# andompesta/nodeembedding-to-communityembedding

Measured on AMD Instinct MI355X. Metric: SGNS pair-updates/sec at d=128, 1M-node graph, higher is better.
Workload: dtype f32

## Files before the change

### nodeembedding-to-communityembedding_amd/csrc/come_sgns_impl.h

```cpp
#pragma once
#include <hip/hip_runtime.h>
#include <stdint.h>

#include "come_internal.h"
#include "come_wave.h"

namespace come {

static __constant__ float c_exp_table[kExpTableSize];

struct LcgLane {
    uint64_t a, c;
};

__device__ inline LcgLane lcg_lane_constants(int k) {
    uint64_t a = 1, c = 0;
    for (int i = 0; i < k; ++i) {
        a = (a * kLcgMul) & kLcgMask;
        c = (c * kLcgMul + kLcgAdd) & kLcgMask;
    }
    return {a, c};
}

__device__ inline uint64_t lcg_next(uint64_t s) { return (s * kLcgMul + kLcgAdd) & kLcgMask; }

struct LcgTable {
    uint64_t a[64], c[64];
};
constexpr LcgTable make_lcg_table() {
    LcgTable t{};
    uint64_t a = 1, c = 0;
    for (int k = 0; k < 64; ++k) {
        t.a[k] = a;
        t.c[k] = c;
        a = (a * kLcgMul) & kLcgMask;
        c = (c * kLcgMul + kLcgAdd) & kLcgMask;
    }
    return t;
}
static __constant__ LcgTable c_lcg = make_lcg_table();
constexpr LcgTable kLcgHost = make_lcg_table();
constexpr uint64_t kLcgA64 = (kLcgHost.a[63] * kLcgMul) & kLcgMask;
constexpr uint64_t kLcgC64 = (kLcgHost.c[63] * kLcgMul + kLcgAdd) & kLcgMask;

struct LcgFromTable {
    int lane;
};
__device__ inline uint64_t lcg_state_of(uint64_t base, const LcgLane &lc) {
    return (lc.a * base + lc.c) & kLcgMask;
}
__device__ inline uint64_t lcg_state_of(uint64_t base, const LcgFromTable &lt) {
    return (c_lcg.a[lt.lane] * base + c_lcg.c[lt.lane]) & kLcgMask;
}

__device__ inline uint32_t table_slot(uint64_t s, uint64_t m, uint32_t d) {
    const uint32_t x = (uint32_t)(s >> 16);
    if (d == 0) return x;
    return (uint32_t)__umul64hi(m * (uint64_t)x, (uint64_t)d);
}

struct PackedWord {
    uint32_t base;
    uint32_t unused;
    uint64_t bits;
};

template <class Args>
__device__ inline uint32_t table_value(const Args &a, uint32_t slot) {
    if (a.packed) {
        const uint4 w = reinterpret_cast<const uint4 *>(a.table)[slot >> 6];
        const uint64_t bits = ((uint64_t)w.w << 32) | w.z;
        const uint64_t mask = (2ull << (slot & 63)) - 1ull;
        return w.x + (uint32_t)__popcll(bits & mask);
    }
    return a.table[slot];
}

__device__ inline int uniform(int v) { return __builtin_amdgcn_readfirstlane(v); }
__device__ inline float uniformf(float v) {
    return __int_as_float(__builtin_amdgcn_readfirstlane(__float_as_int(v)));
}
__device__ inline uint64_t uniform64(uint64_t v) {
    const uint32_t lo = __builtin_amdgcn_readfirstlane((uint32_t)v);
    const uint32_t hi = __builtin_amdgcn_readfirstlane((uint32_t)(v >> 32));
    return ((uint64_t)hi << 32) | lo;
}
__device__ inline uint32_t readlane_u32(uint32_t v, int lane) {
    return (uint32_t)__builtin_amdgcn_readlane((int)v, lane);
}
__device__ inline uint64_t readlane_u64(uint64_t v, int lane) {
    const uint32_t lo = readlane_u32((uint32_t)v, lane);
    const uint32_t hi = readlane_u32((uint32_t)(v >> 32), lane);
    return ((uint64_t)hi << 32) | lo;
}

template <int VEC, bool FULL>
struct Row {
    float v[VEC];

    __device__ inline void load(const float *__restrict__ row, int lane, int d) {
#pragma unroll
        for (int i = 0; i < VEC; ++i) {
            const int e = lane + 64 * i;
            v[i] = (FULL || e < d) ? row[e] : 0.0f;
        }
    }

    __device__ inline void load_nt(const float *__restrict__ row, int lane, int d) {
#pragma unroll
        for (int i = 0; i < VEC; ++i) {
            const int e = lane + 64 * i;
            v[i] = (FULL || e < d) ? __builtin_nontemporal_load(row + e) : 0.0f;
        }
    }

    __device__ inline void load_fresh(const float *__restrict__ row, int lane, int d) {
#pragma unroll
        for (int i = 0; i < VEC; ++i) {
            const int e = lane + 64 * i;
            v[i] = (FULL || e < d) ? __hip_atomic_load(row + e, __ATOMIC_RELAXED,
                                                       __HIP_MEMORY_SCOPE_AGENT)
                                   : 0.0f;
        }
    }

    __device__ inline void load_as(const float *__restrict__ row, int lane, int d, bool fresh) {
        if (fresh) load_fresh(row, lane, d);
        else load(row, lane, d);
    }

    __device__ inline void store(float *__restrict__ row, int lane, int d) const {
#pragma unroll
        for (int i = 0; i < VEC; ++i) {
            const int e = lane + 64 * i;
            if (FULL || e < d) row[e] = v[i];
        }
    }

    __device__ inline void atomic_add(float *__restrict__ row, int lane, int d) const {
#pragma unroll
        for (int i = 0; i < VEC; ++i) {
            const int e = lane + 64 * i;
            if (FULL || e < d) atomicAdd(row + e, v[i]);
        }
    }
};

template <int VEC, bool FULL>
__device__ inline float lane_partial(const Row<VEC, FULL> &a, const Row<VEC, FULL> &b) {
    float p = 0.0f;
#pragma unroll
    for (int i = 0; i < VEC; ++i) p = __builtin_fmaf(a.v[i], b.v[i], p);
    return p;
}

__device__ inline float wave_sum(float p) {
    p = reduce_stage<0>(p);
    p = reduce_stage<1>(p);
    p = reduce_stage<2>(p);
    p = reduce_stage<3>(p);
    p = reduce_stage<4>(p);
    return reduce_stage<5>(p);
}

template <int N>
__device__ inline void wave_sum_n(float (&part)[N], int count) {
#define COME_STAGE(S)                                          \
    _Pragma("unroll") for (int k = 0; k < N; ++k) if (k < count) part[k] = reduce_stage<S>(part[k]);
    COME_STAGE(0) COME_STAGE(1) COME_STAGE(2) COME_STAGE(3) COME_STAGE(4) COME_STAGE(5)
#undef COME_STAGE
}

__device__ inline bool sigmoid_ref(float f, float *sig) {
    if (f <= -(float)kMaxExp || f >= (float)kMaxExp) return false;
    const int b = (int)(((double)f + 6.0) * 83.0);
    *sig = c_exp_table[b];
    return true;
}

__device__ inline bool sigmoid_tab(const float *tab, float f, float *sig) {
    if (f <= -(float)kMaxExp || f >= (float)kMaxExp) return false;
    const int b = (int)(((double)f + 6.0) * 83.0);
    *sig = tab[b];
    return true;
}

struct DrawBatch {
    uint32_t target;
    uint64_t base;
    int used;
};

template <class Args>
__device__ inline void draws_fill(DrawBatch &b, uint64_t state0, const LcgLane &lc,
                                  const Args &a, int count = 64) {
    b.base = state0;
    b.used = 0;
    b.target = 0;
    if ((int)(threadIdx.x & 63) < count) {
        const uint64_t s = (lc.a * state0 + lc.c) & kLcgMask;
        b.target = table_value(a, table_slot(s, a.fm.m, a.fm.d));
    }
}

__device__ inline uint64_t draws_state_at_used(const DrawBatch &b, const LcgLane &lc) {
    const uint64_t s = (lc.a * b.base + lc.c) & kLcgMask;
    if (b.used < 64) return uniform64(readlane_u64(s, b.used));
    return lcg_next(uniform64(readlane_u64(s, 63)));
}

struct DrawPipe {
    uint32_t t0, t1;
    uint64_t base0, base1;
    int used;

    template <class Args, class Lcg>
    __device__ inline uint32_t gather(uint64_t base, const Lcg &lc, const Args &a) {
        const uint64_t s = lcg_state_of(base, lc);
        return table_value(a, table_slot(s, a.fm.m, a.fm.d));
    }

    template <class Args, class Lcg>
    __device__ inline uint32_t gather_hot(uint64_t base, const Lcg &lc, const Args &a) {
        const uint32_t v = gather(base, lc, a);
        if (a.hot == nullptr || (int64_t)v >= a.V) return v;
        return v | (((a.hot[v >> 5] >> (v & 31)) & 1u) << 31);
    }
};


struct O2Args {
    float *node;
    float *ctx;
    const int32_t *walks;
    const uint64_t *seeds;
    const uint32_t *table;
    int64_t V;
    int64_t P;
    int L;
    int d;
    int window;
    int negative;
    float lr;
    float alpha;
    FastMod fm;
    int packed;
    int64_t *counter;
    unsigned long long *upd_count;
    int fresh;
    int wb_atomic;
    const uint32_t *hot;
};

template <class Args>
__device__ inline bool is_hot(const Args &a, int r) {
    return a.hot != nullptr && ((a.hot[(uint32_t)r >> 5] >> (r & 31)) & 1u);
}

__device__ inline int64_t next_unit(int64_t *counter, int64_t cur, int64_t stride, int lane) {
    if (!counter) return cur + stride;
    int64_t v = 0;
    if (lane == 0) v = (int64_t)atomicAdd((unsigned long long *)counter, 1ull);
    return (int64_t)uniform64((uint64_t)v);
}

__device__ inline uint64_t advance64_uniform(uint64_t base) {
    return (kLcgA64 * base + kLcgC64) & kLcgMask;
}
__device__ inline uint64_t advance64(uint64_t base, const LcgLane &lc) {
    const uint64_t s = (lc.a * base + lc.c) & kLcgMask;
    return lcg_next(uniform64(readlane_u64(s, 63)));
}

template <int VEC, bool FULL>
__device__ inline void atomic_add_delta(float *__restrict__ row, const Row<VEC, FULL> &cur,
                                        const Row<VEC, FULL> &orig, int lane, int d) {
    Row<VEC, FULL> delta;
#pragma unroll
    for (int e = 0; e < VEC; ++e) delta.v[e] = cur.v[e] - orig.v[e];
    delta.atomic_add(row, lane, d);
}

template <int VEC, bool FULL, int MAXN>
__device__ inline void o2_pair(const O2Args &a, DrawBatch &db, const LcgLane &lc, int lane, int ci,
                               Row<VEC, FULL> &pos, bool &pos_upd, Row<VEC, FULL> &in,
                               Row<VEC, FULL> &work, int &nupd) {
    using R = Row<VEC, FULL>;
    const int n = a.negative;
    const int d = a.d;
    if (n > 0 && db.used + n > 64) draws_fill(db, draws_state_at_used(db, lc), lc, a);
    int t[MAXN + 1];
    bool valid[MAXN + 1];
    t[0] = ci;
    valid[0] = true;
#pragma unroll
    for (int k = 1; k <= MAXN; ++k) {
        if (k <= n) {
            const int tk = (int)readlane_u32(db.target, db.used + k - 1);
            t[k] = tk;
            valid[k] = tk != ci && tk >= 0 && tk < a.V;
        } else {
            t[k] = -1;
            valid[k] = false;
        }
    }
    if (n > 0) db.used += n;

    R r[MAXN + 1], o[MAXN + 1];
#pragma unroll
    for (int k = 1; k <= MAXN; ++k)
        if (valid[k]) {
            r[k].load_as(a.ctx + (int64_t)t[k] * d, lane, d, a.fresh);
            o[k] = r[k];
        }

    float part[MAXN + 1];
    part[0] = lane_partial(in, pos);
#pragma unroll
    for (int k = 1; k <= MAXN; ++k) part[k] = valid[k] ? lane_partial(in, r[k]) : 0.0f;
    wave_sum_n(part, n + 1);

#pragma unroll
    for (int e = 0; e < VEC; ++e) work.v[e] = 0.0f;
    {
        float sig;
        if (sigmoid_ref(uniformf(part[0]), &sig)) {
            const float g = ((1.0f - sig) * a.lr) * a.alpha;
#pragma unroll
            for (int e = 0; e < VEC; ++e) {
                work.v[e] = __builtin_fmaf(g, pos.v[e], work.v[e]);
                pos.v[e] = __builtin_fmaf(g, in.v[e], pos.v[e]);
            }
            pos_upd = true;
            ++nupd;
        }
    }
    bool upd[MAXN + 1];
    upd[0] = false;
#pragma unroll
    for (int k = 1; k <= MAXN; ++k) {
        upd[k] = false;
        if (!valid[k]) continue;
        float f = part[k];
        int prev = -1;
#pragma unroll
        for (int q = 1; q < k; ++q)
            if (valid[q] && t[q] == t[k]) prev = q;
        if (prev >= 0) {
#pragma unroll
            for (int q = 1; q < k; ++q) {
                if (q == prev) {
                    r[k] = r[q];
                    f = upd[q] ? wave_sum(lane_partial(in, r[k])) : part[q];
                }
            }
        }
        f = uniformf(f);
        part[k] = f;
        float sig;
        if (!sigmoid_ref(f, &sig)) continue;
        const float g = ((0.0f - sig) * a.lr) * a.alpha;
#pragma unroll
        for (int e = 0; e < VEC; ++e) {
            work.v[e] = __builtin_fmaf(g, r[k].v[e], work.v[e]);
            r[k].v[e] = __builtin_fmaf(g, in.v[e], r[k].v[e]);
        }
        upd[k] = true;
        ++nupd;
    }
#pragma unroll
    for (int k = 1; k <= MAXN; ++k) {
        if (!upd[k]) continue;
        if (!a.wb_atomic && !is_hot(a, t[k])) {
            r[k].store(a.ctx + (int64_t)t[k] * d, lane, d);
            continue;
        }
        bool last = true;
#pragma unroll
        for (int q = k + 1; q <= MAXN; ++q)
            if (upd[q] && t[q] == t[k]) last = false;
        if (last) atomic_add_delta(a.ctx + (int64_t)t[k] * d, r[k], o[k], lane, d);
    }
#pragma unroll
    for (int e = 0; e < VEC; ++e) in.v[e] = in.v[e] + work.v[e];
}

template <int VEC, bool FULL, int MAXN>
__global__ void __launch_bounds__(256) k_sgns_o2(O2Args a) {
    using R = Row<VEC, FULL>;
    const int lane = threadIdx.x & 63;
    const int64_t waves_per_block = blockDim.x >> 6;
    const int64_t gw = (int64_t)blockIdx.x * waves_per_block + (threadIdx.x >> 6);
    const int64_t nwaves = (int64_t)gridDim.x * waves_per_block;
    const LcgLane lc = lcg_lane_constants(lane);
    const int d = a.d;
    const int path_len = a.L < kMaxSentenceLen ? a.L : kMaxSentenceLen;

    for (int64_t p = gw; p < a.P; p += nwaves) {
        const int32_t *__restrict__ idx = a.walks + p * (int64_t)a.L;
        DrawBatch db;
        db.used = 0;
        db.base = uniform64(a.seeds[p]);
        db.target = 0;
        if (a.negative > 0) draws_fill(db, db.base, lc, a);
        int nupd = 0;
        for (int i = 0; i < path_len; ++i) {
            const int ci = uniform(idx[i]);
            if (ci < 0 || ci >= a.V) continue;
            const int j0 = i - a.window < 0 ? 0 : i - a.window;
            const int j1 = i + a.window + 1 > path_len ? path_len : i + a.window + 1;
            for (int j = j0; j < j1; ++j) {
                if (j == i) continue;
                const int cj = uniform(idx[j]);
                if (cj < 0 || cj >= a.V) continue;
                R in, pos;
                in.load_as(a.node + (int64_t)cj * d, lane, d, a.fresh);
                pos.load_as(a.ctx + (int64_t)ci * d, lane, d, a.fresh);
                const R pos0 = pos;
                bool pos_upd = false;
                R work;
                o2_pair<VEC, FULL, MAXN>(a, db, lc, lane, ci, pos, pos_upd, in, work, nupd);
                if (pos_upd) {
                    if (a.wb_atomic || is_hot(a, ci))
                        atomic_add_delta(a.ctx + (int64_t)ci * d, pos, pos0, lane, d);
                    else
                        pos.store(a.ctx + (int64_t)ci * d, lane, d);
                }
                if (a.wb_atomic || is_hot(a, cj)) work.atomic_add(a.node + (int64_t)cj * d, lane, d);
                else in.store(a.node + (int64_t)cj * d, lane, d);
            }
        }
        if (a.upd_count && lane == 0 && nupd) atomicAdd(a.upd_count, (unsigned long long)nupd);
    }
}

template <int VEC, bool FULL, int MAXN>
__global__ void __launch_bounds__(128) k_sgns_o2_ring(O2Args a) {
    using R = Row<VEC, FULL>;
    extern __shared__ __attribute__((aligned(16))) float lds[];
    const int lane = threadIdx.x & 63;
    const int wib = threadIdx.x >> 6;
    const int64_t waves_per_block = blockDim.x >> 6;
    const int64_t gw = (int64_t)blockIdx.x * waves_per_block + wib;
    const int64_t nwaves = (int64_t)gridDim.x * waves_per_block;
    const LcgLane lc = lcg_lane_constants(lane);
    const int d = a.d;
    const int w = a.window;
    const int n = a.negative;
    const int RS = 2 * w + 1;
    const int path_len = a.L < kMaxSentenceLen ? a.L : kMaxSentenceLen;
    const int wave_floats = (RS * d + 3) & ~3;
    float *ring = lds + wib * wave_floats;
    auto valid_row = [&](int r) { return r >= 0 && r < a.V; };
    auto slot_add = [&](int s, int delta) {
        s += delta;
        if (s < 0) s += RS;
        if (s >= RS) s -= RS;
        return s;
    };

    for (int64_t p = a.counter ? next_unit(a.counter, 0, 0, lane) : gw; p < a.P;
         p = next_unit(a.counter, p, nwaves, lane)) {
        const int32_t *__restrict__ walk = a.walks + p * (int64_t)a.L;
        int wbase = 0;
        int c0 = lane < path_len ? walk[lane] : -1;
        int c1 = 64 + lane < path_len ? walk[64 + lane] : -1;
        auto idx_at = [&](int q) {
            if (q >= path_len) return -1;
            const int off = q - wbase;
            const int r = off < 64 ? __builtin_amdgcn_readlane(c0, off)
                                   : __builtin_amdgcn_readlane(c1, off - 64);
            return valid_row(r) ? r : -1;
        };
        DrawPipe dp;
        dp.used = 0;
        dp.base0 = uniform64(a.seeds[p]);
        dp.t0 = dp.t1 = 0;
        if (n > 0) {
            dp.t0 = dp.gather(dp.base0, lc, a);
            dp.base1 = advance64(dp.base0, lc);
            dp.t1 = dp.gather(dp.base1, lc, a);
        }
        auto take = [&](int k) -> int {
            const int q = dp.used + k;
            return (int)(q < 64 ? readlane_u32(dp.t0, q) : readlane_u32(dp.t1, q - 64));
        };
        auto advance = [&]() {
            if (n == 0) return;
            dp.used += n;
            if (dp.used >= 64) {
                dp.used -= 64;
                dp.t0 = dp.t1;
                dp.base0 = dp.base1;
                dp.base1 = advance64(dp.base1, lc);
                dp.t1 = dp.gather(dp.base1, lc, a);
            }
        };
        int tn[MAXN + 1];
        R rn[MAXN + 1];
        auto fetch_next = [&]() {
#pragma unroll
            for (int k = 1; k <= MAXN; ++k) {
                const int tk = k <= n ? take(k - 1) : -1;
                tn[k] = tk;
                rn[k].load(a.ctx + (int64_t)(valid_row(tk) ? tk : 0) * d, lane, d);
            }
        };
        fetch_next();

        int nupd = 0;
        int ids = -1;
        auto id_of = [&](int s) { return __builtin_amdgcn_readlane(ids, s); };
        auto alias_mask = [&](int id, int except) -> uint64_t {
            return __ballot(lane < RS && lane != except && ids == id);
        };
        auto set_id = [&](int s, int id) { ids = lane == s ? id : ids; };
        auto write_back = [&](int s, int id) {
            if (alias_mask(id, s) != 0) return;
            R row;
            row.load(ring + s * d, lane, d);
            row.store(a.node + (int64_t)id * d, lane, d);
        };
        auto enter_row = [&](int s, int id, const R &fetched) {
            const uint64_t m = alias_mask(id, s);
            if (m) {
                R row;
                row.load(ring + __builtin_ctzll(m) * d, lane, d);
                row.store(ring + s * d, lane, d);
            } else {
                fetched.store(ring + s * d, lane, d);
            }
            set_id(s, id);
        };
        for (int q = 0; q < w && q < path_len; ++q) {
            const int id = idx_at(q);
            if (id >= 0) {
                R row;
                row.load(a.node + (int64_t)id * d, lane, d);
                enter_row(q, id, row);
            }
        }
        R pos_n, ent_n;
        int pos_n_id = idx_at(0), ent_n_id = idx_at(w);
        pos_n.load(a.ctx + (int64_t)(pos_n_id >= 0 ? pos_n_id : 0) * d, lane, d);
        ent_n.load(a.node + (int64_t)(ent_n_id >= 0 ? ent_n_id : 0) * d, lane, d);

        int si = 0;
        for (int i = 0; i < path_len; ++i) {
            if (i + 1 + w >= wbase + 128) {
                wbase += 64;
                c0 = c1;
                c1 = wbase + 64 + lane < path_len ? walk[wbase + 64 + lane] : -1;
            }
            const int ci = pos_n_id;
            R pos = pos_n;
            const int se = slot_add(si, w);
            if (i + w < path_len || i - w - 1 >= 0) {
                const int old_id = i - w - 1 >= 0 ? id_of(se) : -1;
                if (old_id >= 0 && old_id == ent_n_id) {
                } else {
                    if (old_id >= 0) write_back(se, old_id);
                    set_id(se, -1);
                    if (i + w < path_len && ent_n_id >= 0) enter_row(se, ent_n_id, ent_n);
                }
            }
            pos_n_id = idx_at(i + 1);
            ent_n_id = idx_at(i + 1 + w);
            pos_n.load(a.ctx + (int64_t)(pos_n_id >= 0 ? pos_n_id : 0) * d, lane, d);
            ent_n.load(a.node + (int64_t)(ent_n_id >= 0 ? ent_n_id : 0) * d, lane, d);

            if (ci >= 0) {
                bool pos_upd = false;
                const int j0 = i - w < 0 ? 0 : i - w;
                const int j1 = i + w + 1 > path_len ? path_len : i + w + 1;
                for (int j = j0; j < j1; ++j) {
                    if (j == i) continue;
                    const int sj = slot_add(si, j - i);
                    const int cj = id_of(sj);
                    if (cj < 0) continue;
                    R in;
                    in.load(ring + sj * d, lane, d);
                    int t[MAXN + 1];
                    R r[MAXN + 1];
#pragma unroll
                    for (int k = 1; k <= MAXN; ++k) {
                        t[k] = tn[k];
                        r[k] = rn[k];
                    }
                    advance();
                    fetch_next();

                    bool valid[MAXN + 1];
#pragma unroll
                    for (int k = 1; k <= MAXN; ++k)
                        valid[k] = k <= n && t[k] != ci && valid_row(t[k]);
                    float part[MAXN + 1];
                    part[0] = lane_partial(in, pos);
#pragma unroll
                    for (int k = 1; k <= MAXN; ++k) part[k] = lane_partial(in, r[k]);
                    wave_sum_n(part, n + 1);
                    R work;
#pragma unroll
                    for (int e = 0; e < VEC; ++e) work.v[e] = 0.0f;
                    {
                        float sig;
                        if (sigmoid_ref(uniformf(part[0]), &sig)) {
                            const float g = ((1.0f - sig) * a.lr) * a.alpha;
#pragma unroll
                            for (int e = 0; e < VEC; ++e) {
                                work.v[e] = __builtin_fmaf(g, pos.v[e], work.v[e]);
                                pos.v[e] = __builtin_fmaf(g, in.v[e], pos.v[e]);
                            }
                            pos_upd = true;
                            ++nupd;
                        }
                    }
                    bool upd[MAXN + 1];
#pragma unroll
                    for (int k = 1; k <= MAXN; ++k) {
                        upd[k] = false;
                        if (!valid[k]) continue;
                        float f = part[k];
                        int prev = -1;
#pragma unroll
                        for (int q = 1; q < k; ++q)
                            if (valid[q] && t[q] == t[k]) prev = q;
                        if (prev >= 0) {
#pragma unroll
                            for (int q = 1; q < k; ++q) {
                                if (q == prev) {
                                    r[k] = r[q];
                                    f = upd[q] ? wave_sum(lane_partial(in, r[k])) : part[q];
                                }
                            }
                        }
                        f = uniformf(f);
                        part[k] = f;
                        float sig;
                        if (!sigmoid_ref(f, &sig)) continue;
                        const float g = ((0.0f - sig) * a.lr) * a.alpha;
#pragma unroll
                        for (int e = 0; e < VEC; ++e) {
                            work.v[e] = __builtin_fmaf(g, r[k].v[e], work.v[e]);
                            r[k].v[e] = __builtin_fmaf(g, in.v[e], r[k].v[e]);
                        }
                        upd[k] = true;
                        ++nupd;
                    }
#pragma unroll
                    for (int k = 1; k <= MAXN; ++k) {
                        if (!upd[k]) continue;
                        r[k].store(a.ctx + (int64_t)t[k] * d, lane, d);
#pragma unroll
                        for (int q = 1; q <= MAXN; ++q)
                            if (tn[q] == t[k]) rn[q] = r[k];
                        if (pos_n_id == t[k]) pos_n = r[k];
                    }
#pragma unroll
                    for (int e = 0; e < VEC; ++e) in.v[e] = in.v[e] + work.v[e];
                    uint64_t m = alias_mask(cj, -1);
                    while (m) {
                        const int rr = __builtin_ctzll(m);
                        m &= m - 1;
                        in.store(ring + rr * d, lane, d);
                    }
                }
                if (pos_upd) {
                    pos.store(a.ctx + (int64_t)ci * d, lane, d);
#pragma unroll
                    for (int q = 1; q <= MAXN; ++q)
                        if (tn[q] == ci) rn[q] = pos;
                    if (pos_n_id == ci) pos_n = pos;
                }
            }
            si = slot_add(si, 1);
        }
        const int first = path_len - w - 1 > 0 ? path_len - w - 1 : 0;
        for (int q = first; q < path_len; ++q) {
            const int s = q % RS;
            const int id = id_of(s);
            if (id >= 0) write_back(s, id);
            set_id(s, -1);
        }
        if (a.upd_count && lane == 0 && nupd) atomicAdd(a.upd_count, (unsigned long long)nupd);
    }
}

template <int VEC, int MAXN>
constexpr int stream_waves_per_eu() {
    return (VEC <= 2 && MAXN <= 5) ? 8 : 1;
}

template <int VEC, bool FULL, int MAXN>
__global__ void __launch_bounds__(256)
    __attribute__((amdgpu_waves_per_eu(stream_waves_per_eu<VEC, MAXN>())))
    k_sgns_o2_stream(O2Args a) {
    using R = Row<VEC, FULL>;
    const int lane = threadIdx.x & 63;
    const int64_t waves_per_block = blockDim.x >> 6;
    const int64_t gw = (int64_t)blockIdx.x * waves_per_block + (threadIdx.x >> 6);
    const int64_t nwaves = (int64_t)gridDim.x * waves_per_block;
    const LcgFromTable lc{lane};
    const int d = a.d;
    const int w = a.window;
    const int n = a.negative;
    const int path_len = a.L < kMaxSentenceLen ? a.L : kMaxSentenceLen;
    auto valid_row = [&](int r) { return r >= 0 && r < a.V; };
    constexpr uint32_t kHotBit = 0x80000000u;
    __shared__ float s_exp[kExpTableSize];
    for (int i = threadIdx.x; i < kExpTableSize; i += blockDim.x) s_exp[i] = c_exp_table[i];
    __syncthreads();
    __shared__ uint32_t s_draws[4][128];
    uint32_t *draws = s_draws[threadIdx.x >> 6];
    __shared__ int s_walk[4][128];
    int *wpos = s_walk[threadIdx.x >> 6];

    for (int64_t p = a.counter ? next_unit(a.counter, 0, 0, lane) : gw; p < a.P;
         p = next_unit(a.counter, p, nwaves, lane)) {
        const int32_t *__restrict__ walk = a.walks + p * (int64_t)a.L;
        auto chunk = [&](int q0) {
            const int q = q0 + lane;
            int v = q < path_len ? walk[q] : -1;
            if (!valid_row(v)) return -1;
            if (a.hot != nullptr && ((a.hot[(uint32_t)v >> 5] >> (v & 31)) & 1u))
                v = (int)((uint32_t)v | kHotBit);
            return v;
        };
        int wbase = 0;
        wpos[lane] = chunk(0);
        wpos[64 + lane] = chunk(64);
        __builtin_amdgcn_wave_barrier();
        auto raw_at = [&](int q) {
            if (q >= path_len) return -1;
            while (q - wbase >= 128) {
                wbase += 64;
                wpos[lane] = wpos[64 + lane];
                wpos[64 + lane] = chunk(wbase + 64);
                __builtin_amdgcn_wave_barrier();
            }
            return uniform(wpos[q - wbase]);
        };
        int it_i = 0, it_j = -1;
        auto next_pair = [&](int &ci, int &cj, int &pi, bool &hi, bool &hj) -> bool {
            for (;;) {
                if (it_i >= path_len) return false;
                const int i = it_i;
                const int j0 = i - w < 0 ? 0 : i - w;
                const int j1 = i + w + 1 > path_len ? path_len : i + w + 1;
                if (it_j < j0) it_j = j0;
                const int rci = raw_at(i);
                if (rci == -1 || it_j >= j1) {
                    ++it_i;
                    it_j = -1;
                    continue;
                }
                const int j = it_j++;
                if (j == i) continue;
                const int rcj = raw_at(j);
                if (rcj == -1) continue;
                ci = (int)((uint32_t)rci & ~kHotBit);
                cj = (int)((uint32_t)rcj & ~kHotBit);
                hi = ((uint32_t)rci & kHotBit) != 0;
                hj = ((uint32_t)rcj & kHotBit) != 0;
                pi = i;
                return true;
            }
        };
        DrawPipe dp;
        dp.used = 0;
        dp.base0 = uniform64(a.seeds[p]);
        if (n > 0) {
            draws[lane] = dp.gather_hot(dp.base0, lc, a);
            dp.base1 = advance64_uniform(dp.base0);
            draws[64 + lane] = dp.gather_hot(dp.base1, lc, a);
            __builtin_amdgcn_wave_barrier();
        }
        auto advance = [&]() {
            if (n == 0) return;
            dp.used += n;
            if (dp.used >= 64) {
                dp.used -= 64;
                draws[lane] = draws[64 + lane];
                dp.base0 = dp.base1;
                dp.base1 = advance64_uniform(dp.base1);
                draws[64 + lane] = dp.gather_hot(dp.base1, lc, a);
                __builtin_amdgcn_wave_barrier();
            }
        };
        int nci = -1, ncj = -1, npi = -1;
        bool nhi = false, nhj = false;
        int tn[MAXN + 1];
        R in_n, pos_n, rn[MAXN + 1];
        int prev_i = -1;
        static_assert(MAXN < 32, "the alias test keeps a pair's rows in half a wavefront");
        uint32_t ids = 0xFFFFFFFFu;
        auto prefetch = [&](bool need_pos) {
            in_n.load(a.node + (int64_t)ncj * d, lane, d);
            if (need_pos) pos_n.load(a.ctx + (int64_t)nci * d, lane, d);
            const bool drawn = lane > 32 && lane <= 32 + n;
            const uint32_t nx = drawn ? draws[drawn ? dp.used + lane - 33 : 0] : 0xFFFFFFFFu;
            ids = lane < 32 ? ids : lane == 32 ? (uint32_t)nci : nx;
#pragma unroll
            for (int k = 1; k <= MAXN; ++k) {
                tn[k] = (int)(readlane_u32(ids, 32 + k) & ~kHotBit);
                if (k > n) tn[k] = -1;
                rn[k].load_nt(a.ctx + (int64_t)(valid_row(tn[k]) ? tn[k] : 0) * d, lane, d);
            }
        };
        bool have = next_pair(nci, ncj, npi, nhi, nhj);
        if (have) prefetch(true);
        int nupd = 0;
        R pos;
        bool pos_upd = false;

        while (have) {
            const int ci = nci, cj = ncj, ic = npi;
            const bool hot_ci = nhi, hot_cj = nhj;
            R in = in_n;
            int t[MAXN + 1];
            R r[MAXN + 1];
#pragma unroll
            for (int k = 1; k <= MAXN; ++k) {
                t[k] = tn[k];
                r[k] = rn[k];
            }
            const bool new_center = ic != prev_i;
            if (new_center || hot_ci) pos = pos_n;
            if (new_center) pos_upd = false;
            prev_i = ic;
            ids = (uint32_t)__builtin_amdgcn_permlane32_swap((int)ids, (int)ids, false, false)[1];
            const uint32_t thm = (uint32_t)__ballot((ids & kHotBit) != 0);
            advance();
            have = next_pair(nci, ncj, npi, nhi, nhj);
            if (have) prefetch(npi != ic || nhi);

            const uint32_t idv = ids & ~kHotBit;
            uint64_t alias = __ballot(idv == (uint32_t)ci) & ~(1ull | (1ull << 32));
#pragma unroll
            for (int k = 1; k <= MAXN; ++k)
                alias |= __ballot(idv == (uint32_t)t[k]) & ~(1ull << k);
            const uint64_t negs = (2ull << n) - 2ull;
            const bool plain = have && ncj != cj && alias == 0 &&
                               (__ballot(idv < (uint32_t)a.V) & negs) == negs;

            bool valid[MAXN + 1];
#pragma unroll
            for (int k = 1; k <= MAXN; ++k)
                valid[k] = !plain && k <= n && t[k] != ci && valid_row(t[k]);
            float part[MAXN + 1];
            part[0] = lane_partial(in, pos);
#pragma unroll
            for (int k = 1; k <= MAXN; ++k) part[k] = lane_partial(in, r[k]);
            wave_sum_n(part, n + 1);
            float fv = 0.0f;
#pragma unroll
            for (int k = 0; k <= MAXN; ++k) fv = lane == k ? part[k] : fv;
            auto f_of = [&](int k) {
                return __int_as_float(__builtin_amdgcn_readlane(__float_as_int(fv), k));
            };
            R work;
#pragma unroll
            for (int e = 0; e < VEC; ++e) work.v[e] = 0.0f;
            uint64_t act = 0;
            if (plain) {
                const bool skip = fv <= -(float)kMaxExp || fv >= (float)kMaxExp;
                int b = (int)(((double)fv + 6.0) * 83.0);
                b = (uint32_t)b < (uint32_t)kExpTableSize ? b : 0;
                act = __ballot(!skip) & ((2ull << n) - 1ull);
                fv = (((lane == 0 ? 1.0f : 0.0f) - s_exp[b]) * a.lr) * a.alpha;
            }
            auto g_of = f_of;
            float gpos = 0.0f;
            {
                float sig = 0.0f;
                if (plain ? (act & 1ull) != 0 : sigmoid_tab(s_exp, f_of(0), &sig)) {
                    const float g = plain ? g_of(0) : ((1.0f - sig) * a.lr) * a.alpha;
#pragma unroll
                    for (int e = 0; e < VEC; ++e) {
                        work.v[e] = __builtin_fmaf(g, pos.v[e], work.v[e]);
                        pos.v[e] = __builtin_fmaf(g, in.v[e], pos.v[e]);
                    }
                    pos_upd = true;
                    gpos = g;
                    ++nupd;
                }
            }
            bool upd[MAXN + 1];
            float gk[MAXN + 1];
#pragma unroll
            for (int k = 1; k <= MAXN; ++k) {
                upd[k] = false;
                gk[k] = 0.0f;
                float g;
                if (plain) {
                    if (!((act >> k) & 1ull)) continue;
                    g = g_of(k);
                } else {
                    if (!valid[k]) continue;
                    float f = f_of(k);
                    int prev = -1;
#pragma unroll
                    for (int q = 1; q < k; ++q)
                        if (valid[q] && t[q] == t[k]) prev = q;
                    if (prev >= 0) {
#pragma unroll
                        for (int q = 1; q < k; ++q) {
                            if (q == prev) {
                                r[k] = r[q];
                                f = upd[q] ? uniformf(wave_sum(lane_partial(in, r[k]))) : f_of(q);
                            }
                        }
                        fv = lane == k ? f : fv;
                    }
                    float sig;
                    if (!sigmoid_tab(s_exp, f, &sig)) continue;
                    g = ((0.0f - sig) * a.lr) * a.alpha;
                }
#pragma unroll
                for (int e = 0; e < VEC; ++e) {
                    work.v[e] = __builtin_fmaf(g, r[k].v[e], work.v[e]);
                    r[k].v[e] = __builtin_fmaf(g, in.v[e], r[k].v[e]);
                }
                upd[k] = true;
                gk[k] = g;
                ++nupd;
            }
#pragma unroll
            for (int k = 1; k <= MAXN; ++k) {
                if (!upd[k]) continue;
                if ((thm >> k) & 1u) {
                    R dlt;
#pragma unroll
                    for (int e = 0; e < VEC; ++e) dlt.v[e] = gk[k] * in.v[e];
                    dlt.atomic_add(a.ctx + (int64_t)t[k] * d, lane, d);
                    if (VEC <= 2 && !plain) {
#pragma unroll
                        for (int q = 1; q <= MAXN; ++q)
                            if (tn[q] == t[k])
#pragma unroll
                                for (int e = 0; e < VEC; ++e) rn[q].v[e] += dlt.v[e];
                        if (have && nci == t[k] && (npi != ic || nhi))
#pragma unroll
                            for (int e = 0; e < VEC; ++e) pos_n.v[e] += dlt.v[e];
                    }
                } else {
                    r[k].store(a.ctx + (int64_t)t[k] * d, lane, d);
                    if (VEC <= 2 && !plain) {
#pragma unroll
                        for (int q = 1; q <= MAXN; ++q)
                            if (tn[q] == t[k]) rn[q] = r[k];
                        if (have && nci == t[k] && (npi != ic || nhi)) pos_n = r[k];
                    }
                }
                if (VEC > 2 && !plain) {
#pragma unroll
                    for (int q = 1; q <= MAXN; ++q)
                        if (tn[q] == t[k])
#pragma unroll
                            for (int e = 0; e < VEC; ++e)
                                rn[q].v[e] = __builtin_fmaf(gk[k], in.v[e], rn[q].v[e]);
                    if (have && nci == t[k] && (npi != ic || nhi))
#pragma unroll
                        for (int e = 0; e < VEC; ++e)
                            pos_n.v[e] = __builtin_fmaf(gk[k], in.v[e], pos_n.v[e]);
                }
            }
            if (hot_ci && gpos != 0.0f) {
                R pdl;
#pragma unroll
                for (int e = 0; e < VEC; ++e) pdl.v[e] = gpos * in.v[e];
                pdl.atomic_add(a.ctx + (int64_t)ci * d, lane, d);
                if (!plain)
#pragma unroll
                    for (int q = 1; q <= MAXN; ++q)
                        if (tn[q] == ci)
#pragma unroll
                            for (int e = 0; e < VEC; ++e) rn[q].v[e] += pdl.v[e];
                if (have && nci == ci)
#pragma unroll
                    for (int e = 0; e < VEC; ++e) pos_n.v[e] += pdl.v[e];
            } else if (!hot_ci && pos_upd && (!have || npi != ic)) {
                pos.store(a.ctx + (int64_t)ci * d, lane, d);
                if (!plain)
#pragma unroll
                    for (int q = 1; q <= MAXN; ++q)
                        if (tn[q] == ci) rn[q] = pos;
                if (have && nci == ci) pos_n = pos;
            }
            if (hot_cj) {
                work.atomic_add(a.node + (int64_t)cj * d, lane, d);
            } else {
#pragma unroll
                for (int e = 0; e < VEC; ++e) in.v[e] = in.v[e] + work.v[e];
                in.store(a.node + (int64_t)cj * d, lane, d);
            }
            if (have && ncj == cj)
#pragma unroll
                for (int e = 0; e < VEC; ++e) in_n.v[e] += work.v[e];
        }
        if (a.upd_count && lane == 0 && nupd) atomicAdd(a.upd_count, (unsigned long long)nupd);
    }
}

struct O1Args {
    float *node;
    const int32_t *edges;
    const uint64_t *seeds;
    const uint32_t *table;
    int64_t V;
    int64_t E;
    int d;
    int negative;
    float lr;
    FastMod fm;
    int packed;
    const uint32_t *hot;
    int64_t chunk;
};

template <int VEC, bool FULL, int MAXN>
__global__ void __launch_bounds__(256) k_sgns_o1(O1Args a) {
    using R = Row<VEC, FULL>;
    const int lane = threadIdx.x & 63;
    const int64_t waves_per_block = blockDim.x >> 6;
    const int64_t gw = (int64_t)blockIdx.x * waves_per_block + (threadIdx.x >> 6);
    const int64_t nwaves = (int64_t)gridDim.x * waves_per_block;
    const LcgLane lc = lcg_lane_constants(lane);
    const int n = a.negative;
    const int d = a.d;

    for (int64_t e = gw; e < a.E; e += nwaves) {
        const int u = uniform(a.edges[2 * e]);
        const int v = uniform(a.edges[2 * e + 1]);
        if (u < 0 || u >= a.V || v < 0 || v >= a.V) continue;
        DrawBatch db;
        db.used = 0;
        db.base = uniform64(a.seeds[e]);
        db.target = 0;
        if (n > 0) draws_fill(db, db.base, lc, a, 2 * n);

        int t1[MAXN + 1], t2[MAXN + 1];
        bool v1[MAXN + 1], v2[MAXN + 1];
        t1[0] = v;
        t2[0] = u;
        v1[0] = v2[0] = true;
#pragma unroll
        for (int k = 1; k <= MAXN; ++k) {
            if (k <= n) {
                t1[k] = (int)readlane_u32(db.target, k - 1);
                t2[k] = (int)readlane_u32(db.target, n + k - 1);
                v1[k] = t1[k] != v && t1[k] >= 0 && t1[k] < a.V;
                v2[k] = t2[k] != u && t2[k] >= 0 && t2[k] < a.V;
            } else {
                t1[k] = t2[k] = -1;
                v1[k] = v2[k] = false;
            }
        }
        R in1, in2;
        in1.load(a.node + (int64_t)u * d, lane, d);
        if (v != u) in2.load(a.node + (int64_t)v * d, lane, d);
        const bool hot_u = is_hot(a, u), hot_v = is_hot(a, v);
        R r1[MAXN + 1], r2[MAXN + 1];
#pragma unroll
        for (int k = 1; k <= MAXN; ++k) {
            if (v1[k]) r1[k].load(a.node + (int64_t)t1[k] * d, lane, d);
            if (v2[k]) r2[k].load(a.node + (int64_t)t2[k] * d, lane, d);
        }
        if (v != u) r1[0] = in2; else r1[0] = in1;

        {
            float part[MAXN + 1];
#pragma unroll
            for (int k = 0; k <= MAXN; ++k) part[k] = v1[k] ? lane_partial(in1, r1[k]) : 0.0f;
            wave_sum_n(part, n + 1);
            R work;
#pragma unroll
            for (int q = 0; q < VEC; ++q) work.v[q] = 0.0f;
#pragma unroll
            for (int k = 0; k <= MAXN; ++k) {
                if (!v1[k]) continue;
                float sig;
                if (!sigmoid_ref(uniformf(part[k]), &sig)) continue;
                const float g = ((k == 0 ? 1.0f : 0.0f) - sig) * a.lr;
#pragma unroll
                for (int q = 0; q < VEC; ++q) work.v[q] = __builtin_fmaf(g, r1[k].v[q], work.v[q]);
            }
#pragma unroll
            for (int q = 0; q < VEC; ++q) in1.v[q] = in1.v[q] + work.v[q];
            if (hot_u) work.atomic_add(a.node + (int64_t)u * d, lane, d);
            else in1.store(a.node + (int64_t)u * d, lane, d);
        }
        r2[0] = in1;
        if (v == u) in2 = in1;
        {
            float part[MAXN + 1];
#pragma unroll
            for (int k = 0; k <= MAXN; ++k) part[k] = v2[k] ? lane_partial(in2, r2[k]) : 0.0f;
            wave_sum_n(part, n + 1);
            R work;
#pragma unroll
            for (int q = 0; q < VEC; ++q) work.v[q] = 0.0f;
#pragma unroll
            for (int k = 0; k <= MAXN; ++k) {
                if (!v2[k]) continue;
                float sig;
                if (!sigmoid_ref(uniformf(part[k]), &sig)) continue;
                const float g = ((k == 0 ? 1.0f : 0.0f) - sig) * a.lr;
#pragma unroll
                for (int q = 0; q < VEC; ++q) work.v[q] = __builtin_fmaf(g, r2[k].v[q], work.v[q]);
            }
#pragma unroll
            for (int q = 0; q < VEC; ++q) in2.v[q] = in2.v[q] + work.v[q];
            if (hot_v) work.atomic_add(a.node + (int64_t)v * d, lane, d);
            else in2.store(a.node + (int64_t)v * d, lane, d);
        }
    }
}

template <int VEC, int MAXN>
constexpr int o1_runs_waves_per_eu() {
    return (VEC <= 2 && MAXN <= 5) ? 8 : 1;
}

template <int VEC, bool FULL, int MAXN>
__global__ void __launch_bounds__(256)
    __attribute__((amdgpu_waves_per_eu(o1_runs_waves_per_eu<VEC, MAXN>())))
    k_sgns_o1_runs(O1Args a) {
    using R = Row<VEC, FULL>;
    const int lane = threadIdx.x & 63;
    const int64_t waves_per_block = blockDim.x >> 6;
    const int64_t gw = (int64_t)blockIdx.x * waves_per_block + (threadIdx.x >> 6);
    const int64_t nwaves = (int64_t)gridDim.x * waves_per_block;
    const LcgLane lc = lcg_lane_constants(lane);
    const int n = a.negative;
    const int d = a.d;
    const int64_t nchunks = (a.E + a.chunk - 1) / a.chunk;

    for (int64_t c = gw; c < nchunks; c += nwaves) {
        const int64_t e0 = c * a.chunk;
        const int64_t e1 = e0 + a.chunk < a.E ? e0 + a.chunk : a.E;
        int cu = -1;
        bool hot_cu = false;
        R hu, du;
        auto flush = [&]() {
            if (cu < 0) return;
            if (hot_cu) du.atomic_add(a.node + (int64_t)cu * d, lane, d);
            else hu.store(a.node + (int64_t)cu * d, lane, d);
        };
        for (int64_t e = e0; e < e1; ++e) {
            const int u = uniform(a.edges[2 * e]);
            const int v = uniform(a.edges[2 * e + 1]);
            if (u < 0 || u >= a.V || v < 0 || v >= a.V) continue;
            if (u != cu) {
                flush();
                cu = u;
                hot_cu = is_hot(a, u);
                hu.load(a.node + (int64_t)u * d, lane, d);
#pragma unroll
                for (int q = 0; q < VEC; ++q) du.v[q] = 0.0f;
            }
            DrawBatch db;
            db.used = 0;
            db.base = uniform64(a.seeds[e]);
            db.target = 0;
            if (n > 0) draws_fill(db, db.base, lc, a, 2 * n);
            int t1[MAXN + 1], t2[MAXN + 1];
            bool v1[MAXN + 1], v2[MAXN + 1];
            t1[0] = v;
            t2[0] = u;
            v1[0] = v2[0] = true;
#pragma unroll
            for (int k = 1; k <= MAXN; ++k) {
                if (k <= n) {
                    t1[k] = (int)readlane_u32(db.target, k - 1);
                    t2[k] = (int)readlane_u32(db.target, n + k - 1);
                    v1[k] = t1[k] != v && t1[k] >= 0 && t1[k] < a.V;
                    v2[k] = t2[k] != u && t2[k] >= 0 && t2[k] < a.V;
                } else {
                    t1[k] = t2[k] = -1;
                    v1[k] = v2[k] = false;
                }
            }
            R in2;
            if (v != u) in2.load(a.node + (int64_t)v * d, lane, d);
            const bool hot_v = is_hot(a, v);
            R r1[MAXN + 1], r2[MAXN + 1];
#pragma unroll
            for (int k = 1; k <= MAXN; ++k) {
                if (v1[k]) {
                    if (t1[k] == u) r1[k] = hu;
                    else r1[k].load(a.node + (int64_t)t1[k] * d, lane, d);
                }
                if (v2[k] && t2[k] != v) r2[k].load(a.node + (int64_t)t2[k] * d, lane, d);
            }
            r1[0] = v != u ? in2 : hu;
            {
                float part[MAXN + 1];
#pragma unroll
                for (int k = 0; k <= MAXN; ++k) part[k] = v1[k] ? lane_partial(hu, r1[k]) : 0.0f;
                wave_sum_n(part, n + 1);
                R work;
#pragma unroll
                for (int q = 0; q < VEC; ++q) work.v[q] = 0.0f;
#pragma unroll
                for (int k = 0; k <= MAXN; ++k) {
                    if (!v1[k]) continue;
                    float sig;
                    if (!sigmoid_ref(uniformf(part[k]), &sig)) continue;
                    const float g = ((k == 0 ? 1.0f : 0.0f) - sig) * a.lr;
#pragma unroll
                    for (int q = 0; q < VEC; ++q) work.v[q] = __builtin_fmaf(g, r1[k].v[q], work.v[q]);
                }
#pragma unroll
                for (int q = 0; q < VEC; ++q) {
                    hu.v[q] = hu.v[q] + work.v[q];
                    du.v[q] = du.v[q] + work.v[q];
                }
            }
            r2[0] = hu;
            if (v == u) in2 = hu;
#pragma unroll
            for (int k = 1; k <= MAXN; ++k)
                if (v2[k] && t2[k] == v) r2[k] = in2;
            {
                float part[MAXN + 1];
#pragma unroll
                for (int k = 0; k <= MAXN; ++k) part[k] = v2[k] ? lane_partial(in2, r2[k]) : 0.0f;
                wave_sum_n(part, n + 1);
                R work;
#pragma unroll
                for (int q = 0; q < VEC; ++q) work.v[q] = 0.0f;
#pragma unroll
                for (int k = 0; k <= MAXN; ++k) {
                    if (!v2[k]) continue;
                    float sig;
                    if (!sigmoid_ref(uniformf(part[k]), &sig)) continue;
                    const float g = ((k == 0 ? 1.0f : 0.0f) - sig) * a.lr;
#pragma unroll
                    for (int q = 0; q < VEC; ++q) work.v[q] = __builtin_fmaf(g, r2[k].v[q], work.v[q]);
                }
                if (v == u) {
#pragma unroll
                    for (int q = 0; q < VEC; ++q) {
                        hu.v[q] = hu.v[q] + work.v[q];
                        du.v[q] = du.v[q] + work.v[q];
                    }
                } else {
#pragma unroll
                    for (int q = 0; q < VEC; ++q) in2.v[q] = in2.v[q] + work.v[q];
                    if (hot_v) work.atomic_add(a.node + (int64_t)v * d, lane, d);
                    else in2.store(a.node + (int64_t)v * d, lane, d);
                }
            }
        }
        flush();
    }
}

struct KernelSet {
    void *o2_direct[2][3];
    void *o2_ring[2][3];
    void *o2_stream[2][3];
    void *o1[2][3];
    void *o1_runs[2][3];
};
#define COME_DECLARE_VEC(V) \
    const KernelSet &kernels_vec##V(); \
    hipError_t upload_exp_table_vec##V(const float *host1000);
COME_DECLARE_VEC(1)
COME_DECLARE_VEC(2)
COME_DECLARE_VEC(4)
COME_DECLARE_VEC(8)
#undef COME_DECLARE_VEC

}
```

Before: 1.039 billion.

## Reload prefetched rows from memory on conflicts instead of patching registers

For small VEC, the stream kernel no longer keeps a per-target id array or patches prefetched rows in registers when a written row aliases a prefetched one. It waits for outstanding memory ops and re-reads the affected rows, with pending hot-center atomic deltas added separately. Target ids are now read from the id register on demand, and the wave reduction runs over all slots without a count guard. The aim is lower register pressure and less branchy forwarding code, at the cost of extra vmcnt waits and reloads on non-plain pairs.

Measured after the change: 1.112 billion, median of 6. 1.07x the previous value.

```diff
diff --git a/nodeembedding-to-communityembedding_amd/csrc/come_sgns_impl.h b/nodeembedding-to-communityembedding_amd/csrc/come_sgns_impl.h
--- a/nodeembedding-to-communityembedding_amd/csrc/come_sgns_impl.h
+++ b/nodeembedding-to-communityembedding_amd/csrc/come_sgns_impl.h
@@ -167,6 +167,14 @@
 __device__ inline void wave_sum_n(float (&part)[N], int count) {
 #define COME_STAGE(S)                                          \
     _Pragma("unroll") for (int k = 0; k < N; ++k) if (k < count) part[k] = reduce_stage<S>(part[k]);
+    COME_STAGE(0) COME_STAGE(1) COME_STAGE(2) COME_STAGE(3) COME_STAGE(4) COME_STAGE(5)
+#undef COME_STAGE
+}
+
+template <int N>
+__device__ inline void wave_sum_all(float (&part)[N]) {
+#define COME_STAGE(S) \
+    _Pragma("unroll") for (int k = 0; k < N; ++k) part[k] = reduce_stage<S>(part[k]);
     COME_STAGE(0) COME_STAGE(1) COME_STAGE(2) COME_STAGE(3) COME_STAGE(4) COME_STAGE(5)
 #undef COME_STAGE
 }
@@ -705,8 +713,11 @@
     const int w = a.window;
     const int n = a.negative;
     const int path_len = a.L < kMaxSentenceLen ? a.L : kMaxSentenceLen;
-    auto valid_row = [&](int r) { return r >= 0 && r < a.V; };
+    const uint32_t Vu = (uint32_t)a.V;
+    auto valid_row = [&](int r) { return (uint32_t)r < Vu; };
+    constexpr bool kReread = VEC <= 2;
     constexpr uint32_t kHotBit = 0x80000000u;
+    constexpr int kWaitVm0 = 0x0F70;
     __shared__ float s_exp[kExpTableSize];
     for (int i = threadIdx.x; i < kExpTableSize; i += blockDim.x) s_exp[i] = c_exp_table[i];
     __syncthreads();
@@ -789,11 +800,15 @@
         };
         int nci = -1, ncj = -1, npi = -1;
         bool nhi = false, nhj = false;
-        int tn[MAXN + 1];
         R in_n, pos_n, rn[MAXN + 1];
+        R padd;
+        bool padd_on = false;
         int prev_i = -1;
         static_assert(MAXN < 32, "the alias test keeps a pair's rows in half a wavefront");
         uint32_t ids = 0xFFFFFFFFu;
+        auto next_target = [&](int k) {
+            return k <= n ? (int)(readlane_u32(ids, 32 + k) & ~kHotBit) : -1;
+        };
         auto prefetch = [&](bool need_pos) {
             in_n.load(a.node + (int64_t)ncj * d, lane, d);
             if (need_pos) pos_n.load(a.ctx + (int64_t)nci * d, lane, d);
@@ -802,13 +817,22 @@
             ids = lane < 32 ? ids : lane == 32 ? (uint32_t)nci : nx;
 #pragma unroll
             for (int k = 1; k <= MAXN; ++k) {
-                tn[k] = (int)(readlane_u32(ids, 32 + k) & ~kHotBit);
-                if (k > n) tn[k] = -1;
-                rn[k].load_nt(a.ctx + (int64_t)(valid_row(tn[k]) ? tn[k] : 0) * d, lane, d);
+                const int tk = next_target(k);
+                rn[k].load_nt(a.ctx + (int64_t)(valid_row(tk) ? tk : 0) * d, lane, d);
+            }
+        };
+        auto reread = [&](bool need_pos) {
+            in_n.load_fresh(a.node + (int64_t)ncj * d, lane, d);
+            if (need_pos) pos_n.load_fresh(a.ctx + (int64_t)nci * d, lane, d);
+#pragma unroll
+            for (int k = 1; k <= MAXN; ++k) {
+                const int tk = next_target(k);
+                rn[k].load_fresh(a.ctx + (int64_t)(valid_row(tk) ? tk : 0) * d, lane, d);
             }
         };
         bool have = next_pair(nci, ncj, npi, nhi, nhj);
         if (have) prefetch(true);
+        if (kReread) __builtin_amdgcn_s_waitcnt(kWaitVm0);
         int nupd = 0;
         R pos;
         bool pos_upd = false;
@@ -821,11 +845,16 @@
             R r[MAXN + 1];
 #pragma unroll
             for (int k = 1; k <= MAXN; ++k) {
-                t[k] = tn[k];
+                t[k] = next_target(k);
                 r[k] = rn[k];
             }
             const bool new_center = ic != prev_i;
-            if (new_center || hot_ci) pos = pos_n;
+            if (new_center || hot_ci) {
+                pos = pos_n;
+                if (kReread && padd_on)
+#pragma unroll
+                    for (int e = 0; e < VEC; ++e) pos.v[e] += padd.v[e];
+            }
             if (new_center) pos_upd = false;
             prev_i = ic;
             ids = (uint32_t)__builtin_amdgcn_permlane32_swap((int)ids, (int)ids, false, false)[1];
@@ -841,7 +870,8 @@
                 alias |= __ballot(idv == (uint32_t)t[k]) & ~(1ull << k);
             const uint64_t negs = (2ull << n) - 2ull;
             const bool plain = have && ncj != cj && alias == 0 &&
-                               (__ballot(idv < (uint32_t)a.V) & negs) == negs;
+                               (__ballot(idv < Vu) & negs) == negs &&
+                               !(kReread && nci == ci && npi != ic);
 
             bool valid[MAXN + 1];
 #pragma unroll
@@ -851,7 +881,7 @@
             part[0] = lane_partial(in, pos);
 #pragma unroll
             for (int k = 1; k <= MAXN; ++k) part[k] = lane_partial(in, r[k]);
-            wave_sum_n(part, n + 1);
+            wave_sum_all(part);
             float fv = 0.0f;
 #pragma unroll
             for (int k = 0; k <= MAXN; ++k) fv = lane == k ? part[k] : fv;
@@ -925,6 +955,7 @@
                 gk[k] = g;
                 ++nupd;
             }
+            if (kReread) __builtin_amdgcn_s_waitcnt(kWaitVm0);
 #pragma unroll
             for (int k = 1; k <= MAXN; ++k) {
                 if (!upd[k]) continue;
@@ -933,29 +964,13 @@
 #pragma unroll
                     for (int e = 0; e < VEC; ++e) dlt.v[e] = gk[k] * in.v[e];
                     dlt.atomic_add(a.ctx + (int64_t)t[k] * d, lane, d);
-                    if (VEC <= 2 && !plain) {
-#pragma unroll
-                        for (int q = 1; q <= MAXN; ++q)
-                            if (tn[q] == t[k])
-#pragma unroll
-                                for (int e = 0; e < VEC; ++e) rn[q].v[e] += dlt.v[e];
-                        if (have && nci == t[k] && (npi != ic || nhi))
-#pragma unroll
-                            for (int e = 0; e < VEC; ++e) pos_n.v[e] += dlt.v[e];
-                    }
                 } else {
                     r[k].store(a.ctx + (int64_t)t[k] * d, lane, d);
-                    if (VEC <= 2 && !plain) {
-#pragma unroll
-                        for (int q = 1; q <= MAXN; ++q)
-                            if (tn[q] == t[k]) rn[q] = r[k];
-                        if (have && nci == t[k] && (npi != ic || nhi)) pos_n = r[k];
-                    }
-                }
-                if (VEC > 2 && !plain) {
+                }
+                if (!kReread && !plain) {
 #pragma unroll
                     for (int q = 1; q <= MAXN; ++q)
-                        if (tn[q] == t[k])
+                        if (next_target(q) == t[k])
 #pragma unroll
                             for (int e = 0; e < VEC; ++e)
                                 rn[q].v[e] = __builtin_fmaf(gk[k], in.v[e], rn[q].v[e]);
@@ -965,27 +980,35 @@
                             pos_n.v[e] = __builtin_fmaf(gk[k], in.v[e], pos_n.v[e]);
                 }
             }
+            padd_on = false;
             if (hot_ci && gpos != 0.0f) {
                 R pdl;
 #pragma unroll
                 for (int e = 0; e < VEC; ++e) pdl.v[e] = gpos * in.v[e];
                 pdl.atomic_add(a.ctx + (int64_t)ci * d, lane, d);
-                if (!plain)
-#pragma unroll
-                    for (int q = 1; q <= MAXN; ++q)
-                        if (tn[q] == ci)
-#pragma unroll
-                            for (int e = 0; e < VEC; ++e) rn[q].v[e] += pdl.v[e];
-                if (have && nci == ci)
-#pragma unroll
-                    for (int e = 0; e < VEC; ++e) pos_n.v[e] += pdl.v[e];
+                if (kReread) {
+                    padd = pdl;
+                    padd_on = plain && nci == ci;
+                } else {
+                    if (!plain)
+#pragma unroll
+                        for (int q = 1; q <= MAXN; ++q)
+                            if (next_target(q) == ci)
+#pragma unroll
+                                for (int e = 0; e < VEC; ++e) rn[q].v[e] += pdl.v[e];
+                    if (have && nci == ci)
+#pragma unroll
+                        for (int e = 0; e < VEC; ++e) pos_n.v[e] += pdl.v[e];
+                }
             } else if (!hot_ci && pos_upd && (!have || npi != ic)) {
                 pos.store(a.ctx + (int64_t)ci * d, lane, d);
-                if (!plain)
-#pragma unroll
-                    for (int q = 1; q <= MAXN; ++q)
-                        if (tn[q] == ci) rn[q] = pos;
-                if (have && nci == ci) pos_n = pos;
+                if (!kReread) {
+                    if (!plain)
+#pragma unroll
+                        for (int q = 1; q <= MAXN; ++q)
+                            if (next_target(q) == ci) rn[q] = pos;
+                    if (have && nci == ci) pos_n = pos;
+                }
             }
             if (hot_cj) {
                 work.atomic_add(a.node + (int64_t)cj * d, lane, d);
@@ -994,9 +1017,16 @@
                 for (int e = 0; e < VEC; ++e) in.v[e] = in.v[e] + work.v[e];
                 in.store(a.node + (int64_t)cj * d, lane, d);
             }
-            if (have && ncj == cj)
+            if (kReread) {
+                if (!plain && have) {
+                    __builtin_amdgcn_s_waitcnt(kWaitVm0);
+                    reread(npi != ic || nhi);
+                    __builtin_amdgcn_s_waitcnt(kWaitVm0);
+                }
+            } else if (have && ncj == cj) {
 #pragma unroll
                 for (int e = 0; e < VEC; ++e) in_n.v[e] += work.v[e];
+            }
         }
         if (a.upd_count && lane == 0 && nupd) atomicAdd(a.upd_count, (unsigned long long)nupd);
     }
```
